# EvolvingLMMs-Lab/multimodal-sae

Measured on AMD Instinct MI355X. Metric: tokens/sec through SAE encode+TopK+decode, d=4096 width=131072, higher is better.
Workload: dtype int8 MFMA candidate select + f32 exact re-score/decode (outputs f32-exact); 1 GPU; BASELINE configs[1]: d_model=4096 width=131072 k=32, T=8192 bf16 activations/step resident in HBM, random-init unit-norm f32 weights; k=32, parallelism=single GPU, distinct_batches=4

## Files before the change

multimodal-sae_amd/csrc/encode_rescore.h:

```cpp
#pragma once
#include <type_traits>

#include "encode_defs.h"
#include "encode_sortsel.h"

namespace {

static_assert(MSAE_RESCORE_U * 4 == 64, "one re-scoring batch must be the 64 floats fast_shape_ok() guarantees");
struct RescoreExt { const unsigned char *recs; int G, C, T, stride, valid; };
struct RescoreFm {
  int *count; int *target; unsigned long long *keys; const float *pre; int rcap;
  unsigned long long *cand;
  int *rank;
  int *defer; int all;
};
struct RescoreArgs {
  const float *b_enc;
  const float *tau_vals; int tau_ld, tau_col;
  const int *cnt; const unsigned long long *cand; int cap;
  int T, d, k, r_max;
  int set_feature; float set_value;
  const f32x4 *rowc, *colc;
  float zz12, z2; int i8;
  float zc2;
  float *vals; int32_t *idx; int64_t *idx64; int32_t *status;
  int *flagged; int *n_flagged; int fb_cap;
  int32_t *rows_out;
  int lpr;
  RescoreExt ext;
  RescoreFm fm;
};
constexpr int FM_SORTED = 1 << 30;
constexpr int FM_TARGET_MASK = 0xFFF, FM_PREFIX_SHIFT = 12, FM_PREFIX_MASK = 0xFF;

__host__ __device__ inline int shard_record_bytes(int C) { return C * 12 + 8; }

__host__ __device__ constexpr int lean_key_slots(int nw, int phase) { return nw == 1 ? 256 : (phase == 1 ? 2048 : 512); }

struct RescoreLds {
  int key_slots, nrp;
  unsigned keys, res, ezs, ef, a, total;
  __host__ __device__ RescoreLds(int key_slots_, int nrp_, int ext_cap, int a_floats)
      : key_slots(key_slots_), nrp(nrp_), keys(0u), res(8u * key_slots_), ezs(res + 8u * nrp_), ef(ezs + 4u * ext_cap),
        a(ef + 4u * ext_cap), total(a + 4u * a_floats + 64u) {}
};
__host__ __device__ inline RescoreLds rescore_lds(int nw, int phase, bool lean, int cap, int r_max, bool ext, int a_floats) {
  return RescoreLds(lean ? lean_key_slots(nw, phase) : cap, lean && phase == 1 ? 0 : next_pow2(r_max + 1), ext ? cap : 0, a_floats);
}

template <int NW_, bool EXT_, bool LDSA_, int PHASE_, bool LEAN_>
struct RescoreCfg {
  static constexpr int NW = NW_, PHASE = PHASE_, NT = 64 * NW_, LEAN_KEYS = lean_key_slots(NW_, PHASE_);
  static constexpr bool EXT = EXT_, LDSA = LDSA_, LEAN = LEAN_;
  static_assert(!LEAN || (PHASE != 0 && !EXT && !LDSA), "LEAN: the PHASE kernels of the single-GPU path");
};

struct RescoreToken {
  __device__ __forceinline__ RescoreToken(unsigned char *smem, const RescoreLds &lds)
      : t(blockIdx.x), lane(threadIdx.x), keys(reinterpret_cast<unsigned long long *>(smem + lds.keys)),
        res(reinterpret_cast<unsigned long long *>(smem + lds.res)), ezs(reinterpret_cast<float *>(smem + lds.ezs)),
        ef(reinterpret_cast<int *>(smem + lds.ef)), a_lds(reinterpret_cast<float *>(smem + lds.a)), kcap(lds.key_slots), nrp(lds.nrp) {}
  int t, lane;
  unsigned long long *keys, *res;
  float *ezs; int *ef;
  float *a_lds;
  int kcap, nrp;
  int cnt, n, np;
  float tau;
  f32x4 rc = {0.f, 0.f, 0.f, 0.f};
};

template <class C>
__device__ __forceinline__ void stage_activations(const RescoreToken &tk, const float *__restrict__ a, int d) {
  for (int i = 4 * tk.lane; i < d; i += 4 * C::NT)
    *reinterpret_cast<f32x4 *>(tk.a_lds + i) = *reinterpret_cast<const f32x4 *>(a + i);
}

template <class C>
__device__ __forceinline__ void load_list(const RescoreArgs &p, RescoreToken &tk) {
  const int t = tk.t, lane = tk.lane;
  if constexpr (C::EXT) {
    __shared__ int s_n;
    __shared__ unsigned s_tau;
    const RescoreExt &x = p.ext;
    const int M = x.G * x.C;
    tk.np = next_pow2(M > 2 ? M : 2);
    if (lane == 0) { s_n = 0; s_tau = 0u; }
    __syncthreads();
    int mine = 0;
    for (int i = lane; i < tk.np; i += C::NT) {
      unsigned long long kv = 0ull;
      if (i < M) {
        const int g = i / x.C, j = i - g * x.C;
        const unsigned char *rec = x.recs + ((size_t)g * x.T + t) * x.stride;
        const unsigned long long key = reinterpret_cast<const unsigned long long *>(rec)[j];
        if (key != 0ull) {
          kv = (key & 0xFFFFFFFF00000000ull) | (unsigned)(0x7FFFFFFF - i);
          tk.ef[i] = rank_key_index(key);
          tk.ezs[i] = reinterpret_cast<const float *>(rec + (size_t)x.C * 8)[j];
          ++mine;
        }
      }
      tk.keys[i] = kv;
    }
    if (mine) atomicAdd(&s_n, mine);
    for (int g = lane; g < x.G; g += C::NT) {
      const unsigned char *rec = x.recs + ((size_t)g * x.T + t) * x.stride;
      atomicMax(&s_tau, f32_order_key(*reinterpret_cast<const float *>(rec + (size_t)x.C * 12)));
    }
    __syncthreads();
    tk.n = tk.cnt = s_n;
    tk.tau = f32_from_order_key(s_tau);
  } else {
    tk.cnt = p.cnt[t];
    tk.n = tk.cnt < p.cap ? tk.cnt : p.cap;
    tk.tau = p.tau_vals[(size_t)t * p.tau_ld + p.tau_col];
    tk.rc = p.rowc[t];
    tk.np = next_pow2(tk.n > 2 ? tk.n : 2);
  }
}

template <class C>
struct KeyPrefix {
  static constexpr int PRE_LO = 96, PRE_HI = 128, PRE_MIN = 192, PRE_PK = 32;
  int n_sorted;
  bool partial = false;
  bool presorted = false;
  bool deferred = false;

  __device__ __forceinline__ KeyPrefix(const RescoreArgs &p, const RescoreToken &tk) : n_sorted(tk.n) {
    if constexpr (C::PHASE == 2) presorted = (p.fm.target[tk.t] & FM_SORTED) != 0;
  }

  __device__ __forceinline__ void full_sort(const RescoreArgs &p, const RescoreToken &tk) {
    if constexpr (C::LEAN) { if (tk.np > C::LEAN_KEYS) { deferred = true; return; } }
    if constexpr (!C::EXT) {
      __syncthreads();
      for (int i = tk.lane; i < tk.np; i += C::NT) tk.keys[i] = (i < tk.n) ? p.cand[(size_t)tk.t * p.cap + i] : 0ull;
    }
    if (presorted) __syncthreads();
    else lds_sort_desc_u64<C::NW, (C::NW == 4 && !C::EXT) ? 8 : 0>(tk.keys, tk.np, tk.kcap, tk.lane);
    partial = false;
    n_sorted = tk.n;
  }
  __device__ __forceinline__ void need_full(const RescoreArgs &p, const RescoreToken &tk) {
    if constexpr (C::LEAN) deferred = true; else full_sort(p, tk);
  }
  __device__ __forceinline__ int count_needed(const RescoreArgs &p, const RescoreToken &tk, float v) {
    int c = count_ge(tk.keys, n_sorted, v);
    if (partial && c >= n_sorted) { need_full(p, tk); if (!deferred) c = count_ge(tk.keys, tk.n, v); }
    return c;
  }

  __device__ __forceinline__ void adopt(const RescoreToken &tk, const unsigned long long *src, int have, int slots) {
    for (int i = tk.lane; i < slots; i += C::NT) tk.keys[i] = i < have ? src[i] : 0ull;
    __syncthreads();
    partial = true;
    n_sorted = have;
  }
  __device__ __forceinline__ void preselect(const RescoreArgs &p, const RescoreToken &tk) {
    static_assert(C::NW == 1 && !C::EXT, "one wave holds the list in registers");
    const int n = tk.n, lane = tk.lane;
    if (!(msae_tuning::RESCORE_PRESELECT && !presorted && n > PRE_MIN && n <= 64 * PRE_PK && p.k + 4 <= 64)) return;
    const int nj = (n + 63) >> 6;
    unsigned long long kreg[PRE_PK];
    wave_load_keys<PRE_PK>(kreg, p.cand + (size_t)tk.t * p.cap, n, nj, lane);
    unsigned lo = 0u, hi = 0xFFFFFFFFu;
    int c_sel = -1;
    unsigned thr = 0u;
    while (hi - lo > 1u) {
      const unsigned mid = lo + ((hi - lo) >> 1);
      const int c = wave_count_if<PRE_PK>(kreg, nj, [mid](unsigned long long key) { return (unsigned)(key >> 32) >= mid; });
      if (c > PRE_HI) lo = mid;
      else if (c < PRE_LO) hi = mid;
      else { c_sel = c; thr = mid; break; }
    }
    if (c_sel <= 0) return;
    wave_compact_if<PRE_PK>(kreg, nj, lane, [thr](unsigned long long key) { return (unsigned)(key >> 32) >= thr; },
                            [&tk](unsigned long long key, bool take, int pos) { if (take) tk.keys[pos] = key; });
    for (int i = c_sel + lane; i < PRE_HI; i += C::NT) tk.keys[i] = 0ull;
    lds_sort_desc_u64<1, 2>(tk.keys, PRE_HI, tk.kcap, lane);
    partial = true;
    n_sorted = c_sel;
  }
};

template <class C>
__device__ __forceinline__ int first_round_target(const RescoreArgs &p, const RescoreToken &tk, KeyPrefix<C> &pre, int has_set, int lim) {
  __shared__ float s_cc[C::NT], s_zs[C::NT], s_pick[2];
  const int lane = tk.lane;
  int target = lim;
  const int mt_max = p.k <= 64 ? 64 : C::NT;
  const int mt = tk.n < mt_max ? tk.n : mt_max;
  float my_cc = -__builtin_inff(), my_zs = 0.f;
  if (lane < mt) {
    const unsigned long long key = tk.keys[lane];
    if constexpr (C::EXT) my_zs = tk.ezs[rank_key_index(key)];
    else my_zs = __builtin_sqrtf(band_sq(tk.rc, p.colc[rank_key_index(key)], p.zz12, p.i8 != 0));
    my_cc = f32_from_order_key((unsigned)(key >> 32)) - my_zs;
  }
  s_cc[lane] = my_cc;
  s_zs[lane] = my_zs;
  if (lane < 2) s_pick[lane] = lane == 0 ? -__builtin_inff() : 0.f;
  __syncthreads();
  const int kk = p.k - has_set;
  if (lane < mt && kk >= 1 && kk <= mt) {
    int rank_c = 0, rank_z = 0;
    for (int j = 0; j < mt; ++j) {
      const float cj = s_cc[j], zj = s_zs[j];
      rank_c += (cj > my_cc || (cj == my_cc && j < lane)) ? 1 : 0;
      rank_z += (zj < my_zs || (zj == my_zs && j < lane)) ? 1 : 0;
    }
    if (rank_c == kk - 1) s_pick[0] = my_cc;
    if (rank_z == mt / 2) s_pick[1] = my_zs;
  }
  __syncthreads();
  if (kk >= 1 && kk <= mt && p.z2 > 0.f) {
    const float thr1 = s_pick[0] - GUARD_ZETA * s_pick[1] * __builtin_amdgcn_rsqf(p.z2);
    int n1 = pre.count_needed(p, tk, thr1);
    if (n1 < p.k + 4) n1 = p.k + 4;
    target = n1 < lim ? n1 : lim;
  }
  if constexpr (C::LDSA && C::PHASE == 0) {
    const int rpp = p.lpr > 0 ? C::NT / p.lpr : C::NT;
    const int fill = rpp < lim ? rpp : lim;
    if (target < fill) target = fill;
  }
  return target;
}

template <class C>
__device__ __forceinline__ void phase1_emit(const RescoreArgs &p, const RescoreToken &tk, const KeyPrefix<C> &pre, int target) {
  const int t = tk.t;
  const int save = pre.partial && pre.n_sorted <= p.fm.rcap && pre.n_sorted <= FM_PREFIX_MASK ? pre.n_sorted : 0;
  for (int c = tk.lane; c < (target > save ? target : save); c += C::NT) {
    const unsigned long long key = tk.keys[c];
    p.fm.keys[(size_t)t * p.fm.rcap + c] = key;
    if (c < target) p.fm.rank[(size_t)t * p.fm.rcap + c] = atomicAdd(p.fm.count + rank_key_index(key), 1);
  }
  if (!pre.partial)
    for (int i = tk.lane; i < tk.n; i += C::NT) p.fm.cand[(size_t)t * p.cap + i] = tk.keys[i];
  if (tk.lane == 0) p.fm.target[t] = target | (save << FM_PREFIX_SHIFT) | (pre.partial ? 0 : FM_SORTED);
}

template <class C, int LPR>
__device__ __forceinline__ int rescore_pass(const RescoreArgs &p, const RescoreToken &tk, const float *__restrict__ a,
                                            const float *__restrict__ W_enc, int has_set, int done, int target) {
  constexpr int RPP = C::NT / LPR;
  constexpr int RS_B = 4 * MSAE_RESCORE_U * LPR;
  const int rq = tk.lane / LPR, q = tk.lane % LPR;
  int my_viol = 0;
  for (int c0 = done; c0 < target; c0 += RPP) {
    const int c = c0 + rq;
    const bool active = c < target;
    const unsigned long long key = active ? tk.keys[c] : tk.keys[c0];
    int f = rank_key_index(key);
    float ext_zs = 0.f;
    f32x4 cc = {0.f, 0.f, 0.f, 0.f};
    if constexpr (C::EXT) { ext_zs = tk.ezs[f]; f = tk.ef[f]; }
    else cc = p.colc[f];
    const float upper = f32_from_order_key((unsigned)(key >> 32));
    const float *__restrict__ w = W_enc + (size_t)f * p.d + 4 * q;
    float acc = 0.f;
    f32x4 wa[MSAE_RESCORE_U], wb[MSAE_RESCORE_U];
    auto fetch = [&](f32x4 (&dst)[MSAE_RESCORE_U], int kk) {
#pragma unroll
      for (int u = 0; u < MSAE_RESCORE_U; ++u) dst[u] = *reinterpret_cast<const f32x4 *>(w + kk + 4 * LPR * u);
    };
    auto consume = [&](const f32x4 (&src)[MSAE_RESCORE_U], int kk) {
#pragma unroll
      for (int u = 0; u < MSAE_RESCORE_U; ++u) {
        [[maybe_unused]] f32x4 av;
        if constexpr (C::LDSA) av = *reinterpret_cast<const f32x4 *>(tk.a_lds + kk + 4 * LPR * u + 4 * q);
#pragma unroll
        for (int qq = 0; qq < LPR; ++qq) {
          [[maybe_unused]] const int k0 = kk + 4 * LPR * u + 4 * qq;
          if constexpr (C::LDSA) {
            acc = __builtin_fmaf(av[0], src[u][0], acc);
            acc = __builtin_fmaf(av[1], src[u][1], acc);
            acc = __builtin_fmaf(av[2], src[u][2], acc);
            acc = __builtin_fmaf(av[3], src[u][3], acc);
          } else {
            acc = __builtin_fmaf(a[k0 + 0], src[u][0], acc);
            acc = __builtin_fmaf(a[k0 + 1], src[u][1], acc);
            acc = __builtin_fmaf(a[k0 + 2], src[u][2], acc);
            acc = __builtin_fmaf(a[k0 + 3], src[u][3], acc);
          }
          if constexpr (LPR == 4)
            acc = __int_as_float(__builtin_amdgcn_update_dpp(0, __float_as_int(acc), 0x93, 0xF, 0xF, false));
          if constexpr (LPR == 2)
            acc = __int_as_float(__builtin_amdgcn_update_dpp(0, __float_as_int(acc), 0xB1, 0xF, 0xF, false));
        }
      }
    };
    fetch(wa, 0);
    for (int kk = 0; kk < p.d; kk += 2 * RS_B) {
      const bool has_b = kk + RS_B < p.d;
      if (has_b) fetch(wb, kk + RS_B);
      consume(wa, kk);
      if (kk + 2 * RS_B < p.d) fetch(wa, kk + 2 * RS_B);
      if (has_b) consume(wb, kk + RS_B);
    }
    const float pre = acc + (p.b_enc ? p.b_enc[f] : 0.f);
    if (active && q == 0) {
      tk.res[has_set + c] = result_key(pre, f);
      const float zs2 = C::EXT ? ext_zs * ext_zs : band_sq(tk.rc, cc, p.zz12, p.i8 != 0);
      if (contradicts_model(pre, upper, zs2, p.z2, p.zc2)) my_viol = 1;
    }
  }
  return my_viol;
}
template <class C>
__device__ __forceinline__ int fm_pickup(const RescoreArgs &p, const RescoreToken &tk, int has_set, int target) {
  int my_viol = 0;
  for (int c = tk.lane; c < target; c += C::NT) {
    const unsigned long long key = tk.keys[c];
    const int f = rank_key_index(key);
    const float upper = f32_from_order_key((unsigned)(key >> 32));
    const float pre = p.fm.pre[(size_t)tk.t * p.fm.rcap + c];
    tk.res[has_set + c] = result_key(pre, f);
    if (contradicts_model(pre, upper, band_sq(tk.rc, p.colc[f], p.zz12, p.i8 != 0), p.z2, p.zc2)) my_viol = 1;
  }
  return my_viol;
}

template <class C>
__device__ __forceinline__ bool verify(const RescoreArgs &p, const RescoreToken &tk, KeyPrefix<C> &pre, int has_set, int done,
                                       int lim, bool viol, bool guarded, int &needed, bool &last) {
  const bool have_k = done + has_set >= p.k;
  const float v_k = f32_from_order_key((unsigned)(tk.res[p.k - 1] >> 32));
  const bool list_ok = tk.cnt <= p.cap && tk.tau > 0.f;
  needed = have_k ? pre.count_needed(p, tk, v_k) : tk.n;
  const bool ok = list_ok && have_k && !viol && needed <= done && v_k > tk.tau * 1.000001f && !guarded;
  last = ok || viol || guarded || done >= lim || !list_ok;
  return ok;
}

template <class C>
__device__ __forceinline__ void defer_token(const RescoreArgs &p, const RescoreToken &tk) {
  if (tk.lane == 0) p.fm.defer[(size_t)(C::PHASE - 1) * p.T + tk.t] = 1;
}

template <class C>
__device__ __forceinline__ void write_token(const RescoreArgs &p, const RescoreToken &tk, bool ok, bool viol, bool guarded,
                                            int has_set, int done, int rounds, int first_target) {
  const int t = tk.t;
  for (int j = tk.lane; j < p.k; j += C::NT) {
    const unsigned long long key = tk.res[j];
    const int fi = key ? rank_key_index(key) : 0;
    if (p.idx) p.idx[(size_t)t * p.k + j] = fi;
    if (p.idx64) p.idx64[(size_t)t * p.k + j] = fi;
    p.vals[(size_t)t * p.k + j] = key ? f32_from_order_key((unsigned)(key >> 32)) : 0.f;
  }
  if (tk.lane == 0) {
    const int reason = 2 | (tk.cnt > p.cap ? 4 : 0) | (!(tk.tau > 0.f) ? 8 : 0) |
                       (done + has_set < p.k ? 16 : 0) | (guarded ? 128 : (viol ? 64 : 32));
    if (p.status) p.status[t] = ok ? 0 : reason;
    if (p.rows_out) p.rows_out[t] = ok ? (C::PHASE == 2 ? 1 << 30 : 0) | ((rounds & 0x3F) << 24) | ((first_target < 0xFFF ? first_target : 0xFFF) << 12) | (done < 0xFFF ? done : 0xFFF) : 0;
    if (!ok) {
      const int slot = atomicAdd(p.n_flagged, 1);
      if (slot < p.fb_cap) p.flagged[slot] = t;
    }
  }
}

template <int NW, bool EXT = false, bool LDSA = false, int PHASE = 0, bool LEAN = false>
__global__ __launch_bounds__(64 * NW) void select_rescore_kernel(RescoreArgs p, const float *__restrict__ a32,
                                                            const float *__restrict__ W_enc) {
  using C = RescoreCfg<NW, EXT, LDSA, PHASE, LEAN>;
  extern __shared__ __attribute__((aligned(16))) unsigned char smem[];
  RescoreToken tk(smem, rescore_lds(NW, PHASE, LEAN, p.cap, p.r_max, EXT, LDSA ? p.d : 0));
  const int t = tk.t, lane = tk.lane;
  if constexpr (EXT) { if (t >= p.ext.valid) return; }
  if constexpr (PHASE != 0 && !LEAN) { if (!p.fm.all && p.fm.defer[(size_t)(PHASE - 1) * p.T + t] == 0) return; }
  MSAE_RTL(0);
  const float *__restrict__ a = a32 + (size_t)t * p.d;
  if constexpr (LDSA && PHASE == 0) stage_activations<C>(tk, a, p.d);
  load_list<C>(p, tk);
  if constexpr (PHASE != 1) { for (int i = lane; i < tk.nrp; i += C::NT) tk.res[i] = 0ull; }
  MSAE_RTL(1);

  KeyPrefix<C> pre(p, tk);
  if constexpr (PHASE == 2 && NW == 1) {
    const int saved = (p.fm.target[t] >> FM_PREFIX_SHIFT) & FM_PREFIX_MASK;
    if (!pre.presorted && saved > 0) pre.adopt(tk, p.fm.keys + (size_t)t * p.fm.rcap, saved, pre.PRE_HI);
  }
  if constexpr (PHASE == 2 && LEAN) {
    if (pre.presorted && tk.n > C::LEAN_KEYS) pre.adopt(tk, p.cand + (size_t)t * p.cap, C::LEAN_KEYS, C::LEAN_KEYS);
  }
  if constexpr (!EXT && NW == 1) { if (!pre.partial) pre.preselect(p, tk); }
  if (!pre.partial) pre.full_sort(p, tk);
  if constexpr (LEAN) { if (pre.deferred) { defer_token<C>(p, tk); return; } }
  MSAE_RTL(2);
  const int has_set = p.set_feature >= 0 ? 1 : 0;
  if constexpr (PHASE != 1) { if (lane == 0 && has_set) tk.res[0] = rank_key(p.set_value, p.set_feature); }

  const int lim = tk.n < p.r_max ? tk.n : p.r_max;
  int target;
  if constexpr (PHASE == 2) target = p.fm.target[t] & FM_TARGET_MASK;
  else target = first_round_target<C>(p, tk, pre, has_set, lim);
  if constexpr (LEAN) { if (pre.deferred) { defer_token<C>(p, tk); return; } }
  MSAE_RTL(3);
  const bool guarded = !EXT && tk.rc[3] != 0.f;
  if (guarded) target = 0;
  if constexpr (PHASE == 1) {
    if (pre.partial && target > pre.n_sorted) pre.need_full(p, tk);
    if constexpr (LEAN) { if (pre.deferred) { defer_token<C>(p, tk); return; } }
    phase1_emit<C>(p, tk, pre, target);
    return;
  }

  int done = 0, rounds = 0;
  bool ok = false, viol = false;
  const int first_target = target;
  for (;;) {
    ++rounds;
    if (pre.partial && target > pre.n_sorted) pre.need_full(p, tk);
    if constexpr (LEAN) { if (pre.deferred) { defer_token<C>(p, tk); return; } }
    int my_viol = 0;
    bool from_fm = false;
    if constexpr (PHASE == 2) {
      if (rounds == 1) { my_viol = fm_pickup<C>(p, tk, has_set, target); from_fm = true; }
    }
    if (!from_fm) {
      if constexpr (LDSA && PHASE == 2) { if (rounds == 2) { stage_activations<C>(tk, a, p.d); __syncthreads(); } }
      const bool few = rounds > 1 && target - done <= C::NT / 4;
      int lpr = few ? 4 : (MSAE_RESCORE_LPR == 4 ? 4 : p.lpr);
      while (lpr > 1 && p.d % (4 * MSAE_RESCORE_U * lpr) != 0) lpr >>= 1;
      if (lpr == 4) my_viol = rescore_pass<C, 4>(p, tk, a, W_enc, has_set, done, target);
      else if (lpr == 2) my_viol = rescore_pass<C, 2>(p, tk, a, W_enc, has_set, done, target);
      else my_viol = rescore_pass<C, 1>(p, tk, a, W_enc, has_set, done, target);
    }
    done = target;
    viol = viol || (__syncthreads_or(my_viol) != 0);
    MSAE_RTL(2 + 2 * rounds);
    lds_sort_desc_u64<NW, NW == 1 ? 1 : 4>(tk.res, next_pow2(done + has_set > 2 ? done + has_set : 2), tk.nrp, lane);
    MSAE_RTL(3 + 2 * rounds);
    int needed;
    bool last;
    ok = verify<C>(p, tk, pre, has_set, done, lim, viol, guarded, needed, last);
    if constexpr (LEAN) { if (pre.deferred) { defer_token<C>(p, tk); return; } }
    if (last) break;
    if constexpr (LEAN) { defer_token<C>(p, tk); return; }
    target = needed > done ? needed : done + 1;
    if (target > lim) target = lim;
    __syncthreads();
  }

  MSAE_RTL(14);
  MSAE_RTL_VALUE(15, ((unsigned long long)rounds << 32) | (unsigned)done);
  write_token<C>(p, tk, ok, viol, guarded, has_set, done, rounds, first_target);
}

constexpr int FM_SCAN_BLOCK = 1024;
__device__ __forceinline__ int fm_pad(int c, int G) { return (c + G - 1) & ~(G - 1); }
__global__ __launch_bounds__(256) void fm_blocksum_kernel(const int *__restrict__ counts, int N, int G, int *__restrict__ bsum) {
  __shared__ int red[4];
  const int i0 = blockIdx.x * FM_SCAN_BLOCK + threadIdx.x * 4;
  int s = 0;
#pragma unroll
  for (int e = 0; e < 4; ++e) s += (i0 + e < N) ? fm_pad(counts[i0 + e], G) : 0;
#pragma unroll
  for (int off = 32; off > 0; off >>= 1) s += __shfl_xor(s, off, 64);
  if ((threadIdx.x & 63) == 0) red[threadIdx.x >> 6] = s;
  __syncthreads();
  if (threadIdx.x == 0) bsum[blockIdx.x] = red[0] + red[1] + red[2] + red[3];
}
__global__ __launch_bounds__(256) void fm_scan_kernel(int *__restrict__ counts, int N, int G, const int *__restrict__ bsum,
                                                      int2 *__restrict__ slots) {
  __shared__ int part[256];
  __shared__ int s_base;
  const int tid = threadIdx.x, b = blockIdx.x;
  int pre = 0;
  for (int j = tid; j < b; j += 256) pre += bsum[j];
  part[tid] = pre;
  __syncthreads();
  if (tid < 64) {
    int v = part[tid] + part[tid + 64] + part[tid + 128] + part[tid + 192];
#pragma unroll
    for (int off = 32; off > 0; off >>= 1) v += __shfl_xor(v, off, 64);
    if (tid == 0) s_base = v;
  }
  __syncthreads();
  const int i0 = b * FM_SCAN_BLOCK + tid * 4;
  int c[4], sum = 0;
#pragma unroll
  for (int e = 0; e < 4; ++e) { c[e] = (i0 + e < N) ? counts[i0 + e] : 0; sum += fm_pad(c[e], G); }
  part[tid] = sum;
  __syncthreads();
  for (int off = 1; off < 256; off <<= 1) {
    const int v = tid >= off ? part[tid - off] : 0;
    __syncthreads();
    part[tid] += v;
    __syncthreads();
  }
  int run = s_base + part[tid] - sum;
#pragma unroll
  for (int e = 0; e < 4; ++e) {
    if (i0 + e < N) {
      counts[i0 + e] = run;
      const int padded = fm_pad(c[e], G);
      for (int q = c[e]; q < padded; ++q) slots[run + q] = make_int2(i0 + e, -1);
      run += padded;
    }
  }
  if (b == (int)gridDim.x - 1 && tid == 255) counts[N] = s_base + part[255];
}
__global__ __launch_bounds__(256) void fm_scatter_kernel(const int *__restrict__ fm_target, const unsigned long long *__restrict__ fm_keys,
                                                         const int *__restrict__ fm_rank, int rcap, const int *__restrict__ starts,
                                                         int2 *__restrict__ slots) {
  const int t = blockIdx.x, target = fm_target[t] & FM_TARGET_MASK;
  for (int c = threadIdx.x; c < target; c += 256) {
    const int f = rank_key_index(fm_keys[(size_t)t * rcap + c]);
    slots[starts[f] + fm_rank[(size_t)t * rcap + c]] = make_int2(f, t * rcap + c);
  }
}
template <int G, int SH>
__device__ __forceinline__ void fma_share(float &acc, float a, float w) {
  if constexpr (G == 16) {
    if constexpr (SH == 0) asm("s_nop 1\n\tv_fmac_f32_dpp %0, %1, %2 row_newbcast:0 row_mask:0xf bank_mask:0xf" : "+v"(acc) : "v"(w), "v"(a));
    else asm("v_fmac_f32_dpp %0, %1, %2 row_newbcast:%3 row_mask:0xf bank_mask:0xf" : "+v"(acc) : "v"(w), "v"(a), "n"(SH));
  } else {
    if constexpr (SH == 0) asm("s_nop 1\n\tv_fmac_f32_dpp %0, %1, %2 quad_perm:[0,0,0,0] row_mask:0xf bank_mask:0xf" : "+v"(acc) : "v"(w), "v"(a));
    else asm("v_fmac_f32_dpp %0, %1, %2 quad_perm:[%3,%3,%3,%3] row_mask:0xf bank_mask:0xf" : "+v"(acc) : "v"(w), "v"(a), "n"(SH));
  }
}
template <int DT, bool HAS_BD, int G, int P, int SH = 0>
struct FmChain {
  template <class WR, class XR>
  static __device__ __forceinline__ void run(float &acc, const WR &sw, const XR &sx, const float *__restrict__ bd) {
    if constexpr (SH < G) {
#pragma unroll
      for (int c = 0; c < 4; ++c) {
        const int e = (P * G + SH) * 4 + c;
        float xf;
        if constexpr (DT == MSAE_F32) xf = __uint_as_float(sx[e >> 2][e & 3]);
        else {
          const unsigned pk = sx[e >> 3][(e >> 1) & 3];
          if constexpr (DT == MSAE_BF16) xf = __uint_as_float((e & 1) ? (pk & 0xFFFF0000u) : (pk << 16));
          else xf = f16_bits_to_f32((unsigned short)((e & 1) ? (pk >> 16) : (pk & 0xFFFFu)));
        }
        float a = xf;
        if constexpr (HAS_BD) a = xf - bd[e];
        fma_share<G, SH>(acc, a, sw[P][c]);
      }
      FmChain<DT, HAS_BD, G, P, SH + 1>::run(acc, sw, sx, bd);
    }
  }
};
template <int DT, int G>
__global__ __launch_bounds__(64) void fm_dot_kernel(const void *__restrict__ x, const float *__restrict__ b_dec,
                                                    const float *__restrict__ W_enc, const float *__restrict__ b_enc,
                                                    const int2 *__restrict__ slots, const int *__restrict__ n_slots_p, int d, int rcap,
                                                    float *__restrict__ fm_pre) {
  const int n_slots = *n_slots_p;
  if ((int)blockIdx.x * 64 >= n_slots) return;
  const int lane = threadIdx.x, slot = blockIdx.x * 64 + lane;
  const int2 fo = slot < n_slots ? slots[slot] : make_int2(slots[n_slots - 1].x, -1);
  const bool valid = fo.y >= 0;
  constexpr bool X32 = DT == MSAE_F32;
  constexpr int KB = 64, WP = KB / (4 * G), XP = X32 ? KB / 4 : KB / 8;
  const float *__restrict__ w = W_enc + (size_t)fo.x * d + 4 * (lane % G);
  const unsigned char *__restrict__ xr = static_cast<const unsigned char *>(x) + (size_t)(valid ? fo.y / rcap : 0) * d * (X32 ? 4 : 2);
  f32x4 wa[WP], wb[WP];
  u32x4 xa[XP], xb[XP];
  float acc = 0.f;
  auto fetch = [&](f32x4 (&dw)[WP], u32x4 (&dx)[XP], int kk) {
#pragma unroll
    for (int p = 0; p < WP; ++p) dw[p] = *reinterpret_cast<const f32x4 *>(w + kk + 4 * G * p);
    if (valid) {
#pragma unroll
      for (int u = 0; u < XP; ++u) dx[u] = *reinterpret_cast<const u32x4 *>(xr + (size_t)kk * (X32 ? 4 : 2) + 16 * u);
    }
  };
  auto walk = [&](auto bd_tag) {
    constexpr bool HAS_BD = decltype(bd_tag)::value;
    auto consume = [&](const f32x4 (&sw)[WP], const u32x4 (&sx)[XP], int kk) {
      const float *__restrict__ bd = HAS_BD ? b_dec + kk : nullptr;
      FmChain<DT, HAS_BD, G, 0>::run(acc, sw, sx, bd);
      if constexpr (WP >= 2) FmChain<DT, HAS_BD, G, 1>::run(acc, sw, sx, bd);
      if constexpr (WP >= 4) { FmChain<DT, HAS_BD, G, 2>::run(acc, sw, sx, bd); FmChain<DT, HAS_BD, G, 3>::run(acc, sw, sx, bd); }
    };
    fetch(wa, xa, 0);
    for (int kk = 0; kk < d; kk += 2 * KB) {
      const bool has_b = kk + KB < d;
      if (has_b) fetch(wb, xb, kk + KB);
      consume(wa, xa, kk);
      if (kk + 2 * KB < d) fetch(wa, xa, kk + 2 * KB);
      if (has_b) consume(wb, xb, kk + KB);
    }
  };
  if (b_dec) walk(std::true_type()); else walk(std::false_type());
  if (valid) fm_pre[fo.y] = acc + (b_enc ? b_enc[fo.x] : 0.f);
}
static_assert(64 / (4 * 16) == 1 && 64 / (4 * 4) == 4, "fm_dot_kernel's consume covers WP = 1, 2 and 4");

struct PackArgs {
  const int *cnt; const unsigned long long *cand; int cap;
  const float *tau_vals; int tau_ld, tau_col;
  const f32x4 *rowc, *colc; float zz12; int i8;
  int C, row_offset, stride;
  unsigned char *recs;
};
template <int PK>
__global__ __launch_bounds__(64) void pack_candidates_kernel(PackArgs p) {
  const int t = blockIdx.x, lane = threadIdx.x;
  const int cnt = p.cnt[t];
  const int n = cnt < p.cap ? cnt : p.cap;
  const float tau = p.tau_vals[(size_t)t * p.tau_ld + p.tau_col];
  const bool bounded = cnt <= p.cap && tau > 0.f && p.rowc[t][3] == 0.f;
  const int nj = bounded ? (n + 63) >> 6 : 0;
  unsigned long long kreg[PK];
  wave_load_keys<PK>(kreg, p.cand + (size_t)t * p.cap, n, nj, lane);
  unsigned long long lo = 0ull, hi = ~0ull;
  if (n > p.C) {
    while (hi - lo > 1ull) {
      const unsigned long long mid = lo + ((hi - lo) >> 1);
      const int c = wave_count_if<PK>(kreg, nj, [mid](unsigned long long key) { return key >= mid; });
      if (c >= p.C) lo = mid; else hi = mid;
    }
  } else {
    lo = 1ull;
  }
  unsigned char *rec = p.recs + (size_t)t * p.stride;
  unsigned long long *okeys = reinterpret_cast<unsigned long long *>(rec);
  float *ozs = reinterpret_cast<float *>(rec + (size_t)p.C * 8);
  const f32x4 rc = p.rowc[t];
  unsigned long long below = 0ull;
  const int taken = wave_compact_if<PK>(
      kreg, nj, lane, [lo](unsigned long long key) { return key >= lo && key != 0ull; },
      [&](unsigned long long key, bool take, int pos) {
        if (take) {
          const int f = rank_key_index(key);
          okeys[pos] = (key & 0xFFFFFFFF00000000ull) | (unsigned)(0x7FFFFFFF - (f + p.row_offset));
          ozs[pos] = __builtin_sqrtf(band_sq(rc, p.colc[f], p.zz12, p.i8 != 0));
        } else {
          below = key > below ? key : below;
        }
      });
  for (int jj = taken + lane; jj < p.C; jj += 64) { okeys[jj] = 0ull; ozs[jj] = 0.f; }
#pragma unroll
  for (int off = 32; off > 0; off >>= 1) {
    const unsigned long long o = __shfl_xor(below, off, 64);
    below = o > below ? o : below;
  }
  if (lane == 0) {
    float b = __builtin_inff();
    if (bounded) b = below != 0ull ? f32_from_order_key((unsigned)(below >> 32)) : tau;
    float *tail = reinterpret_cast<float *>(rec + (size_t)p.C * 12);
    tail[0] = b;
    tail[1] = 0.f;
  }
}

inline void rescore_shape(int T, int k, int &nw, int &lpr) {
  nw = k <= 64 ? 1 : 4;
  lpr = 1;
  if (k <= 64) {
    const long lanes = (long)T * (k + 13);
    if (T <= 256 && lanes * 4 <= 131072) lpr = 4;
    else if (T <= 640 && lanes * 2 <= 131072) lpr = 2;
    if (const char *e = getenv("MSAE_LPR")) { const int v = atoi(e); if (v == 1 || v == 2 || v == 4) lpr = v; }
    nw = lpr;
  }
}

template <int NW, bool EXT, bool LDSA, int PHASE, bool LEAN>
inline int launch_rescore_kernel(const RescoreArgs &ra, const RescoreLds &lds, const float *a32, const float *W_enc, hipStream_t s) {
  const auto kernel = select_rescore_kernel<NW, EXT, LDSA, PHASE, LEAN>;
  MSAE_HIP_TRY(hipFuncSetAttribute((const void *)kernel, hipFuncAttributeMaxDynamicSharedMemorySize, (int)lds.total));
  hipLaunchKernelGGL(kernel, dim3(ra.T), dim3(64 * NW), lds.total, s, ra, a32, W_enc);
  return 0;
}
template <bool EXT, int PHASE = 0>
inline int launch_select_rescore(RescoreArgs &ra, const float *a32, const float *W_enc, hipStream_t s) {
  int nw;
  rescore_shape(ra.T, ra.k, nw, ra.lpr);
  auto lds = [&](bool lean, bool with_a) { return rescore_lds(nw, PHASE, lean, ra.cap, ra.r_max, EXT, with_a ? ra.d : 0); };
  const RescoreLds full = lds(false, false), full_a = lds(false, true);
  if constexpr (PHASE != 0) {
    const RescoreLds lean = lds(true, false);
    const bool has_lean = ra.fm.defer != nullptr && lean.total < full.total && (nw == 1 || PHASE == 2 || ra.cap >= 2048);
    ra.fm.all = has_lean ? 0 : 1;
    if (has_lean) {
      const int rc = nw == 1 ? launch_rescore_kernel<1, EXT, false, PHASE, true>(ra, lean, a32, W_enc, s)
                             : launch_rescore_kernel<4, EXT, false, PHASE, true>(ra, lean, a32, W_enc, s);
      if (rc) return rc;
    }
    if constexpr (PHASE == 2) {
      if (nw == 1 && full_a.total <= 64 * 1024) return launch_rescore_kernel<1, EXT, true, 2, false>(ra, full_a, a32, W_enc, s);
    }
    if (nw == 1) return launch_rescore_kernel<1, EXT, false, PHASE, false>(ra, full, a32, W_enc, s);
    return launch_rescore_kernel<4, EXT, false, PHASE, false>(ra, full, a32, W_enc, s);
  } else {
    const bool ldsa = ra.lpr > 1 && full_a.total <= 96 * 1024;
    if (ldsa && nw == 2) return launch_rescore_kernel<2, EXT, true, 0, false>(ra, full_a, a32, W_enc, s);
    if (ldsa) return launch_rescore_kernel<4, EXT, true, 0, false>(ra, full_a, a32, W_enc, s);
    if (nw == 1) return launch_rescore_kernel<1, EXT, false, 0, false>(ra, full, a32, W_enc, s);
    if (nw == 2) return launch_rescore_kernel<2, EXT, false, 0, false>(ra, full, a32, W_enc, s);
    return launch_rescore_kernel<4, EXT, false, 0, false>(ra, full, a32, W_enc, s);
  }
}

inline bool fm_pays(int T, int k, int N, int d, int esize) {
  const char *e = getenv("MSAE_FM");
  const int force = e ? atoi(e) : -1;
  if (force >= 0) return force != 0;
  const double m = 1.36 * (double)T * k / N;
  if (m < 0.6) return false;
  const double tm_rate = m >= 2.0 ? 6.2 : 4.2;
  const double gain_ps = d * (4.0 / tm_rate - (esize + 4.0 / m) / 8.0);
  return gain_ps >= 500.0;
}
inline int fm_group_lanes(int T, int k, int N) { return 1.36 * (double)T * k >= 12.0 * N ? 16 : 4; }
inline bool fm_shape_ok(int T, int k, int N, int d, int r_max) {
  int nw, lpr;
  rescore_shape(T, k, nw, lpr);
  if (lpr != 1 || r_max > 0xFFF || (long)T * r_max + (long)N * 16 >= (1L << 31)) return false;
  return fm_pays(T, k, N, d, 2);
}

}
```

multimodal-sae_amd/csrc/encode_sortsel.h:

```cpp
#pragma once
#include "common.h"

namespace {

template <int NT>
__device__ __forceinline__ void wave_sort_desc_u64(unsigned long long *s, int n, int lane) {
  for (int size = 2; size <= n; size <<= 1)
    for (int stride = size >> 1; stride > 0; stride >>= 1) {
      __syncthreads();
      for (int i = lane; i < (n >> 1); i += NT) {
        const int lo = (i / stride) * (stride << 1) + (i % stride), hi = lo + stride;
        const bool desc = ((lo & size) == 0);
        const unsigned long long x = s[lo], y = s[hi];
        if ((x < y) == desc) { s[lo] = y; s[hi] = x; }
      }
    }
  __syncthreads();
}

template <int R>
__device__ __forceinline__ void wave_sort_desc_u64_regs(unsigned long long (&v)[R], int lane) {
#pragma unroll
  for (int size = 2; size <= 64 * R; size <<= 1)
#pragma unroll
    for (int stride = size >> 1; stride > 0; stride >>= 1) {
      if (stride >= 64) {
        const int rs = stride >> 6;
#pragma unroll
        for (int r = 0; r < R; ++r) {
          if ((r & rs) == 0) {
            const bool desc = (((r * 64 + lane) & size) == 0);
            const unsigned long long a = v[r], b = v[r | rs];
            if ((a < b) == desc) { v[r] = b; v[r | rs] = a; }
          }
        }
      } else {
#pragma unroll
        for (int r = 0; r < R; ++r) {
          const int i = r * 64 + lane;
          const unsigned lo = __shfl_xor((unsigned)v[r], stride, 64), hi = __shfl_xor((unsigned)(v[r] >> 32), stride, 64);
          const unsigned long long o = ((unsigned long long)hi << 32) | lo;
          const bool lower = (lane & stride) == 0, desc = ((i & size) == 0);
          const bool take_max = lower == desc;
          v[r] = take_max ? (v[r] > o ? v[r] : o) : (v[r] < o ? v[r] : o);
        }
      }
    }
}

template <int NW, int R>
__device__ __forceinline__ void wg_sort_desc_u64_regs(unsigned long long (&v)[R], int tid, unsigned long long *xch) {
  constexpr int M = 64 * NW * R;
#pragma unroll
  for (int size = 2; size <= M; size <<= 1)
#pragma unroll
    for (int stride = size >> 1; stride > 0; stride >>= 1) {
      if (stride < R) {
#pragma unroll
        for (int r = 0; r < R; ++r) {
          if ((r & stride) == 0) {
            const bool desc = (((tid * R + r) & size) == 0);
            const unsigned long long a = v[r], b = v[r | stride];
            if ((a < b) == desc) { v[r] = b; v[r | stride] = a; }
          }
        }
      } else {
        const int pt = stride / R;
        const bool lower = (tid & pt) == 0;
        if (pt >= 64) {
          __syncthreads();
#pragma unroll
          for (int r = 0; r < R; ++r) xch[tid * R + r] = v[r];
          __syncthreads();
        }
#pragma unroll
        for (int r = 0; r < R; ++r) {
          unsigned long long o;
          if (pt >= 64) o = xch[(tid ^ pt) * R + r];
          else o = ((unsigned long long)__shfl_xor((unsigned)(v[r] >> 32), pt, 64) << 32) | __shfl_xor((unsigned)v[r], pt, 64);
          const bool desc = (((tid * R + r) & size) == 0);
          const bool take_max = lower == desc;
          v[r] = take_max ? (v[r] > o ? v[r] : o) : (v[r] < o ? v[r] : o);
        }
      }
    }
}

template <int NW, int R>
__device__ __forceinline__ void lds_sort_desc_u64_regs(unsigned long long *s, int n, int tid) {
  __syncthreads();
  unsigned long long v[R];
  const auto at = [tid](int r) { return NW == 1 ? r * 64 + tid : tid * R + r; };
#pragma unroll
  for (int r = 0; r < R; ++r) v[r] = at(r) < n ? s[at(r)] : 0ull;
  if constexpr (NW == 1) wave_sort_desc_u64_regs<R>(v, tid);
  else { wg_sort_desc_u64_regs<NW, R>(v, tid, s); __syncthreads(); }
#pragma unroll
  for (int r = 0; r < R; ++r) s[at(r)] = v[r];
  __syncthreads();
}

template <int NW, int RMAX>
__device__ __forceinline__ void lds_sort_desc_u64(unsigned long long *s, int n, int slots, int tid) {
  if constexpr (NW == 1 && RMAX >= 1) { if (n <= 64 && slots >= 64) { lds_sort_desc_u64_regs<1, 1>(s, n, tid); return; } }
  if constexpr (NW == 1 && RMAX >= 2) { if (n <= 128 && slots >= 128) { lds_sort_desc_u64_regs<1, 2>(s, n, tid); return; } }
  if constexpr (NW == 4 && RMAX >= 4) { if (n <= 1024 && slots >= 1024) { lds_sort_desc_u64_regs<4, 4>(s, n, tid); return; } }
  if constexpr (NW == 4 && RMAX >= 8) { if (n <= 2048 && slots >= 2048) { lds_sort_desc_u64_regs<4, 8>(s, n, tid); return; } }
  wave_sort_desc_u64<64 * NW>(s, n < slots ? n : slots, tid);
}

__device__ __forceinline__ int count_ge(const unsigned long long *keys, int n, float v) {
  const unsigned tk = f32_order_key(v);
  int lo = 0, hi = n;
  while (lo < hi) {
    const int mid = (lo + hi) >> 1;
    if ((unsigned)(keys[mid] >> 32) >= tk) lo = mid + 1; else hi = mid;
  }
  return lo;
}

template <int PK>
__device__ __forceinline__ void wave_load_keys(unsigned long long (&kreg)[PK], const unsigned long long *__restrict__ src, int n,
                                               int nj, int lane) {
#pragma unroll
  for (int j = 0; j < PK; ++j) kreg[j] = (j < nj && j * 64 + lane < n) ? src[j * 64 + lane] : 0ull;
}
template <int PK, class Pred>
__device__ __forceinline__ int wave_count_if(const unsigned long long (&kreg)[PK], int nj, Pred pred) {
  static_assert(PK % 8 == 0, "eight key slots per branch");
  int c = 0;
#pragma unroll
  for (int jb = 0; jb < PK; jb += 8) {
    if (jb < nj) {
#pragma unroll
      for (int j = jb; j < jb + 8; ++j) c += __builtin_popcountll(__builtin_amdgcn_ballot_w64(pred(kreg[j])));
    }
  }
  return c;
}
template <int PK, class Pred, class Visit>
__device__ __forceinline__ int wave_compact_if(const unsigned long long (&kreg)[PK], int nj, int lane, Pred pred, Visit visit) {
  int base = 0;
#pragma unroll
  for (int j = 0; j < PK; ++j) {
    if (j < nj) {
      const bool take = pred(kreg[j]);
      const unsigned long long m = __builtin_amdgcn_ballot_w64(take);
      visit(kreg[j], take, base + __builtin_popcountll(m & ((1ull << lane) - 1ull)));
      base += __builtin_popcountll(m);
    }
  }
  return base;
}

}
```

Baseline: 1.571 million tokens/s.

## Shrink lean rescore register and LDS footprint to raise occupancy

The single-wave preselect now keeps only the 32-bit high halves of the candidate keys in registers and reloads the full 64-bit key from global memory only for the candidates it keeps. Lean single-wave kernels cap their result-slot LDS area at 256 entries. Phase-2 tokens whose target would overflow that area are deferred. Lean kernels also get a launch-bounds occupancy hint of 8 waves. The aim is to cut VGPR and LDS pressure so more waves fit per CU, at the cost of extra global reloads and possibly more deferred tokens.

Result: no change. 1.571 million tokens/s, median of 3 (+0.0%).

```diff
diff --git a/multimodal-sae_amd/csrc/encode_rescore.h b/multimodal-sae_amd/csrc/encode_rescore.h
--- a/multimodal-sae_amd/csrc/encode_rescore.h
+++ b/multimodal-sae_amd/csrc/encode_rescore.h
@@ -44,8 +44,11 @@
       : key_slots(key_slots_), nrp(nrp_), keys(0u), res(8u * key_slots_), ezs(res + 8u * nrp_), ef(ezs + 4u * ext_cap),
         a(ef + 4u * ext_cap), total(a + 4u * a_floats + 64u) {}
 };
+constexpr int LEAN_RES_SLOTS = 256;
 __host__ __device__ inline RescoreLds rescore_lds(int nw, int phase, bool lean, int cap, int r_max, bool ext, int a_floats) {
-  return RescoreLds(lean ? lean_key_slots(nw, phase) : cap, lean && phase == 1 ? 0 : next_pow2(r_max + 1), ext ? cap : 0, a_floats);
+  int nrp = lean && phase == 1 ? 0 : next_pow2(r_max + 1);
+  if (lean && nw == 1 && nrp > LEAN_RES_SLOTS) nrp = LEAN_RES_SLOTS;
+  return RescoreLds(lean ? lean_key_slots(nw, phase) : cap, nrp, ext ? cap : 0, a_floats);
 }
 
 template <int NW_, bool EXT_, bool LDSA_, int PHASE_, bool LEAN_>
@@ -163,21 +166,22 @@
     const int n = tk.n, lane = tk.lane;
     if (!(msae_tuning::RESCORE_PRESELECT && !presorted && n > PRE_MIN && n <= 64 * PRE_PK && p.k + 4 <= 64)) return;
     const int nj = (n + 63) >> 6;
-    unsigned long long kreg[PRE_PK];
-    wave_load_keys<PRE_PK>(kreg, p.cand + (size_t)tk.t * p.cap, n, nj, lane);
+    const unsigned long long *__restrict__ src = p.cand + (size_t)tk.t * p.cap;
+    unsigned vreg[PRE_PK];
+    wave_load_values<PRE_PK>(vreg, src, n, nj, lane);
     unsigned lo = 0u, hi = 0xFFFFFFFFu;
     int c_sel = -1;
     unsigned thr = 0u;
     while (hi - lo > 1u) {
       const unsigned mid = lo + ((hi - lo) >> 1);
-      const int c = wave_count_if<PRE_PK>(kreg, nj, [mid](unsigned long long key) { return (unsigned)(key >> 32) >= mid; });
+      const int c = wave_count_if<PRE_PK>(vreg, nj, [mid](unsigned v) { return v >= mid; });
       if (c > PRE_HI) lo = mid;
       else if (c < PRE_LO) hi = mid;
       else { c_sel = c; thr = mid; break; }
     }
     if (c_sel <= 0) return;
-    wave_compact_if<PRE_PK>(kreg, nj, lane, [thr](unsigned long long key) { return (unsigned)(key >> 32) >= thr; },
-                            [&tk](unsigned long long key, bool take, int pos) { if (take) tk.keys[pos] = key; });
+    wave_compact_if<PRE_PK>(vreg, nj, lane, [thr](unsigned v) { return v >= thr; },
+                            [&tk, src, lane](unsigned, bool take, int pos, int j) { if (take) tk.keys[pos] = src[j * 64 + lane]; });
     for (int i = c_sel + lane; i < PRE_HI; i += C::NT) tk.keys[i] = 0ull;
     lds_sort_desc_u64<1, 2>(tk.keys, PRE_HI, tk.kcap, lane);
     partial = true;
@@ -365,7 +369,7 @@
 }
 
 template <int NW, bool EXT = false, bool LDSA = false, int PHASE = 0, bool LEAN = false>
-__global__ __launch_bounds__(64 * NW) void select_rescore_kernel(RescoreArgs p, const float *__restrict__ a32,
+__global__ __launch_bounds__(64 * NW, LEAN ? 8 : 1) void select_rescore_kernel(RescoreArgs p, const float *__restrict__ a32,
                                                             const float *__restrict__ W_enc) {
   using C = RescoreCfg<NW, EXT, LDSA, PHASE, LEAN>;
   extern __shared__ __attribute__((aligned(16))) unsigned char smem[];
@@ -403,6 +407,7 @@
   MSAE_RTL(3);
   const bool guarded = !EXT && tk.rc[3] != 0.f;
   if (guarded) target = 0;
+  if constexpr (PHASE == 2 && LEAN) { if (target + has_set > tk.nrp) { defer_token<C>(p, tk); return; } }
   if constexpr (PHASE == 1) {
     if (pre.partial && target > pre.n_sorted) pre.need_full(p, tk);
     if constexpr (LEAN) { if (pre.deferred) { defer_token<C>(p, tk); return; } }
@@ -629,7 +634,7 @@
   unsigned long long below = 0ull;
   const int taken = wave_compact_if<PK>(
       kreg, nj, lane, [lo](unsigned long long key) { return key >= lo && key != 0ull; },
-      [&](unsigned long long key, bool take, int pos) {
+      [&](unsigned long long key, bool take, int pos, int) {
         if (take) {
           const int f = rank_key_index(key);
           okeys[pos] = (key & 0xFFFFFFFF00000000ull) | (unsigned)(0x7FFFFFFF - (f + p.row_offset));
diff --git a/multimodal-sae_amd/csrc/encode_sortsel.h b/multimodal-sae_amd/csrc/encode_sortsel.h
--- a/multimodal-sae_amd/csrc/encode_sortsel.h
+++ b/multimodal-sae_amd/csrc/encode_sortsel.h
@@ -125,8 +125,15 @@
 #pragma unroll
   for (int j = 0; j < PK; ++j) kreg[j] = (j < nj && j * 64 + lane < n) ? src[j * 64 + lane] : 0ull;
 }
-template <int PK, class Pred>
-__device__ __forceinline__ int wave_count_if(const unsigned long long (&kreg)[PK], int nj, Pred pred) {
+template <int PK>
+__device__ __forceinline__ void wave_load_values(unsigned (&vreg)[PK], const unsigned long long *__restrict__ src, int n, int nj,
+                                                 int lane) {
+#pragma unroll
+  for (int j = 0; j < PK; ++j)
+    vreg[j] = (j < nj && j * 64 + lane < n) ? reinterpret_cast<const unsigned *>(src + j * 64 + lane)[1] : 0u;
+}
+template <int PK, class K, class Pred>
+__device__ __forceinline__ int wave_count_if(const K (&kreg)[PK], int nj, Pred pred) {
   static_assert(PK % 8 == 0, "eight key slots per branch");
   int c = 0;
 #pragma unroll
@@ -138,15 +145,15 @@
   }
   return c;
 }
-template <int PK, class Pred, class Visit>
-__device__ __forceinline__ int wave_compact_if(const unsigned long long (&kreg)[PK], int nj, int lane, Pred pred, Visit visit) {
+template <int PK, class K, class Pred, class Visit>
+__device__ __forceinline__ int wave_compact_if(const K (&kreg)[PK], int nj, int lane, Pred pred, Visit visit) {
   int base = 0;
 #pragma unroll
   for (int j = 0; j < PK; ++j) {
     if (j < nj) {
       const bool take = pred(kreg[j]);
       const unsigned long long m = __builtin_amdgcn_ballot_w64(take);
-      visit(kreg[j], take, base + __builtin_popcountll(m & ((1ull << lane) - 1ull)));
+      visit(kreg[j], take, base + __builtin_popcountll(m & ((1ull << lane) - 1ull)), j);
       base += __builtin_popcountll(m);
     }
   }
```
